# secondmind-labs/markovflow

Measured on AMD Instinct MI355X. Metric: Kalman log-lik steps/sec (BxT) at d=6, higher is better.
Workload: dtype f64; 1 GPU; KalmanFilter.log_likelihood B=1024/GPU T=10000 d=6 m=1 f64 (sum of two Matern-5/2, north-star target config); series_per_gpu=1024, state_dim=6, output_dim=1, parallelism=batch-sharded x1, one scalar RCCL all-reduce

## Files before the change

### markovflow_amd/csrc/mf_inst.hip

```cpp
#ifndef MF_D
#error "compile with -DMF_D=<state dimension>"
#endif
#include "mf_kernels.hpp"
#include "mf_kf_lds.hpp"
#include "mf_kf_x.hpp"
#include "mf_row.hpp"
#include "mf_row_par.hpp"
#include "mf_row_scan.hpp"
#include "mf_row_grad.hpp"
#include "mf_row_post.hpp"
#include "mf_row_gpr.hpp"
#include "mf_btd_par.hpp"
#include "mf_gpr_fused.hpp"
#include "mf_kl_grad.hpp"
#include "mf_post.hpp"
#include "mf_launch.hpp"

#include <cstdlib>
#include <string>
#include <type_traits>

namespace mf {
namespace {

// ... 73 lines not shown
    return v;
}

template <typename T> bool x_path() {
    static const bool on = [] { const char* e = mf_knob("MF_KF_X"); return !(e && e[0] == '0'); }();
    return on && ((sizeof(T) == 8 && D >= 7) || (sizeof(T) == 4 && D >= 9));
}
template <typename T> bool x_obs_lds(int m) {
    const int a = LdsSpike<T, D>::BYTES, b = a + LdsObs<T, D>::bytes(m);
    return (160 * 1024) / b >= 1 && ((160 * 1024) / b == (160 * 1024) / a || (160 * 1024) / b >= 4);
}
template <typename T> long x_target_lanes() {
    int w = (160 * 1024) / LdsSpike<T, D>::BYTES;
    w = w > 4 ? 4 : (w < 1 ? 1 : w);
    return 256L * 64 * w;
}

template <typename T>
int reduce_levels(RedSys<T> cur, long B, char* p, T add_const, T* out, int* info, hipStream_t st) {
    while (cur.n > red_final()) {
        const long P = cdiv(cur.n, red_chunk());
        RedSys<T> nxt = carve<T>(p, B, P);
        const long lanes = B * P;
        constexpr int x_lds = LdsSpike<T, D>::BYTES;
        if (x_path<T>())
            MF_LANE_LAUNCH((red_chunk_x_kernel<T, D>), dim3((unsigned)cdiv(lanes, 64)), dim3(64), x_lds, st, cur, nxt, B,
                               P, info);
        else
            MF_LANE_LAUNCH((red_chunk_kernel<T, D, true>), dim3((unsigned)cdiv(lanes, 64)), dim3(64), 0, st, cur, nxt,
                               B, P, info);
        cur = nxt;
    }
    MF_LANE_LAUNCH((red_final_kernel<T, D>), dim3((unsigned)cdiv(B, 64)), dim3(64), 0, st, cur, B, add_const, out,
                       info);
    return hipGetLastError() == hipSuccess ? 0 : -1000;
}

constexpr bool ROW_RED_SMALL = D >= 4 && D <= 6;
template <typename T>
int reduce_levels_row(RedSys<T> cur, long B, char* p, T add_const, T* out, int* info, hipStream_t st) {
    if constexpr ((D >= 7 || ROW_RED_SMALL) && D + 1 <= 16) {
        while (cur.n > row_red_final()) {
            const long P = cdiv(cur.n, row_red_chunk());
            RedSys<T> nxt = carve<T>(p, B, P);
            hipLaunchKernelGGL((row::red_row_kernel<T, D>), dim3((unsigned)cdiv(B * P, 4)), dim3(64), 0, st, cur, nxt, B, P, info);
            cur = nxt;
        }
        hipLaunchKernelGGL((row::red_row_final_kernel<T, D>), dim3((unsigned)cdiv(B, 4)), dim3(64), 0, st, cur, B, add_const, out,
                           info);
    }
    return hipGetLastError() == hipSuccess ? 0 : -1000;
}

template <typename T, int M, bool RSTEP> constexpr bool lds_supported() { return KfLdsCfg<T, D, M, RSTEP>::SUPPORTED; }
template <typename T> bool use_lds_kernel(long Tn, int m, int rinv_per_step) {
    static const bool force_direct = [] {
        const char* e = mf_knob("MF_KF_IMPL");
        return e && std::string(e) == "direct";
    }();
    if (force_direct || Tn < 2) return false;
    if (rinv_per_step) return m == 1 && lds_supported<T, 1, true>();
    switch (m) {
        case 1: return lds_supported<T, 1, false>();
        case 2: return lds_supported<T, 2, false>();
        case 3: return lds_supported<T, 3, false>();
        case 4: return lds_supported<T, 4, false>() && (sizeof(T) == 4 || D <= 5);
        default: return false;
    }
}
template <typename T> long lds_target_lanes(int m, int rinv_per_step) {
    auto waves = [](int lds_bytes) { const int w = (160 * 1024) / lds_bytes; return w > 4 ? 4 : (w < 1 ? 1 : w); };
    int w = 4;
    if (rinv_per_step) w = waves(KfLdsCfg<T, D, 1, true>::LDS_TOTAL);
    else if (m == 2) w = waves(KfLdsCfg<T, D, 2, false>::LDS_TOTAL);
    else if (m == 3) w = waves(KfLdsCfg<T, D, 3, false>::LDS_TOTAL);
    else if (m == 4) w = waves(KfLdsCfg<T, D, 4, false>::LDS_TOTAL);
    long lanes = 256L * 64 * w;
    const long small = sizeof(T) == 8 ? (D <= 3 ? 32768L : 65536L) : (D <= 3 ? 32768L : (D <= 5 ? 49152L : 65536L));
    return lanes < small ? lanes : small;
}

inline void lds_partition(long B, long Tn, long chunks, long& P, long& L, long target_lanes = 65536) {
    const long nt = Tn - 1;
    long want = chunks > 0 ? chunks : auto_chunks(B, nt);
    if (chunks <= 0 && target_lanes < 65536) {
        want = cdiv(target_lanes, B);
        const long maxP = nt / 4 > 0 ? nt / 4 : 1;
        if (want > maxP) want = maxP;
    }
    if (want > nt) want = nt;
    if (want < 1) want = 1;
    L = cdiv(nt, want);
    P = cdiv(nt, L);
}

enum KfPath { KF_PATH_ROW, KF_PATH_X, KF_PATH_LDS, KF_PATH_DIRECT };
template <typename T> bool row_path() {
    static const bool on = [] { const char* e = mf_knob("MF_KF_ROW"); return !(e && e[0] == '0'); }();
    return on && D + 1 <= 16 && ((sizeof(T) == 8 && D >= 7) || (sizeof(T) == 4 && D >= 9));
}
template <typename T> long row_target_rows() {
    static const long v = [] {
        const char* e = mf_knob("MF_ROW_TARGET");
        const long x = e ? std::atol(e) : 0;
        const int waves = (sizeof(T) == 4 || D <= 9) ? 3 : row::row_waves_per_simd(D);
        return x > 0 ? x : 256L * 4 * waves * 4;
    }();
    return v;
}
struct KfPlan {
    KfPath path;
    long P, L;
};
inline bool row_reduction(KfPath path) { return path == KF_PATH_ROW || (ROW_RED_SMALL && path == KF_PATH_LDS); }
template <typename T> size_t plan_ws(long B, const KfPlan& pl) {
    return row_reduction(pl.path) ? levels_ws<T>(B, pl.P, row_red_chunk(), row_red_final()) : levels_ws<T>(B, pl.P);
}
template <typename T> KfPlan kf_plan(long B, long Tn, int m, int rinv_per_step, long chunks, bool aligned16) {
    KfPlan pl{KF_PATH_DIRECT, 1, 0};
    if (row_path<T>() && Tn >= 2 && m >= 1 && m <= ROW_MAXM) {
        long P = chunks > 0 ? (chunks > Tn ? Tn : chunks) : cdiv(row_target_rows<T>(), B);
        if (chunks <= 0) {
            const long maxP = Tn / 4 > 0 ? Tn / 4 : 1;
            if (P > maxP) P = maxP;
        }
        if (row::row_offsets_fit(Tn, P, D, m, (int)sizeof(T))) {
            pl.path = KF_PATH_ROW;
            pl.P = P;
            return pl;
// ... 47 lines not shown
    const KfPlan pl = kf_plan<T>(B, Tn, m, rinv_per_step, chunks, aligned16);
    const long P = pl.P;
    if constexpr (!LANE) { if (pl.path != KF_PATH_ROW) return -100; }
    if (ws_bytes < plan_ws<T>(B, pl)) return -15;
    int dbg = 0;
#ifdef MF_EXPERIMENT
    static const int dbg_env = [] { const char* e = mf_knob("MF_KF_DEBUG"); return e ? std::atoi(e) : 0; }();
    dbg = dbg_env;
#endif
    KfArgs<T> a{B, Tn, m, mu0, cholP0, A, b, cholQ, H, y, Rinv, rinv_per_step, P, info, dbg};
    char* p = static_cast<char*>(ws);
    RedSys<T> lvl0 = carve<T>(p, B, P);
    const dim3 grid((unsigned)cdiv(B * P, 64)), block(64);
    if (ev0) (void)hipEventRecord(ev0, st);
    if (pl.path == KF_PATH_ROW) {
        if constexpr (D >= 7 && D + 1 <= 16) {
            const dim3 rgrid((unsigned)cdiv(B * P, 4));
            auto launch = [&](auto mtag) {
                constexpr int M = decltype(mtag)::value;
                if (rinv_per_step) hipLaunchKernelGGL((row::kf_row_kernel<T, D, M, true>), rgrid, block, 0, st, a, lvl0);
                else hipLaunchKernelGGL((row::kf_row_kernel<T, D, M, false>), rgrid, block, 0, st, a, lvl0);
            };
            using std::integral_constant;
            if (m == 1) launch(integral_constant<int, 1>{});
            else if (m == 2) launch(integral_constant<int, 2>{});
            else if (m == 3) launch(integral_constant<int, 3>{});
            else if (m == 4) launch(integral_constant<int, 4>{});
            else if constexpr (!LANE) {
                if (m == 5) launch(integral_constant<int, 5>{});
                else if (m == 6) launch(integral_constant<int, 6>{});
                else if (m == 7) launch(integral_constant<int, 7>{});
                else launch(integral_constant<int, 8>{});
            }
        }
    } else if (pl.path == KF_PATH_X) {
        constexpr int x_lds = LdsSpike<T, D>::BYTES;
        if (m > 1 && x_obs_lds<T>(m)) {
            const int lds = x_lds + LdsObs<T, D>::bytes(m);
            if constexpr (LANE) if (lds > 64 * 1024) {
                static const hipError_t raised = hipFuncSetAttribute(
                    reinterpret_cast<const void*>(&kf_chunk_x_kernel<T, D, true>), hipFuncAttributeMaxDynamicSharedMemorySize,
                    x_lds + LdsObs<T, D>::bytes(MF_MAXM));
                if (raised != hipSuccess) return -1000;
            }
            MF_LANE_LAUNCH((kf_chunk_x_kernel<T, D, true>), grid, block, lds, st, a, lvl0);
        } else {
            MF_LANE_LAUNCH((kf_chunk_x_kernel<T, D, false>), grid, block, x_lds, st, a, lvl0);
        }
    } else if (pl.path == KF_PATH_LDS) {
        const long L = pl.L;
        auto launch = [&](auto mtag, auto rtag) {
            constexpr int M = decltype(mtag)::value;
            constexpr bool RS = decltype(rtag)::value;
            if constexpr (KfLdsCfg<T, D, M, RS>::SUPPORTED) {
                constexpr int lds = KfLdsCfg<T, D, M, RS>::LDS_TOTAL;
                if (P > 1) MF_LANE_LAUNCH((kf_chunk_lds_kernel<T, D, M, true, RS>), grid, block, lds, st, a, L, lvl0);
                else MF_LANE_LAUNCH((kf_chunk_lds_kernel<T, D, M, false, RS>), grid, block, lds, st, a, L, lvl0);
            }
        };
        using std::integral_constant;
        if (rinv_per_step) launch(integral_constant<int, 1>{}, integral_constant<bool, true>{});
        else if (m == 1) launch(integral_constant<int, 1>{}, integral_constant<bool, false>{});
        else if (m == 2) launch(integral_constant<int, 2>{}, integral_constant<bool, false>{});
        else if (m == 3) launch(integral_constant<int, 3>{}, integral_constant<bool, false>{});
        else launch(integral_constant<int, 4>{}, integral_constant<bool, false>{});
    } else if (P > 1) {
        if (m == 1) MF_LANE_LAUNCH((kf_chunk_kernel<T, D, 1, true>), grid, block, 0, st, a, lvl0);
        else MF_LANE_LAUNCH((kf_chunk_kernel<T, D, 0, true>), grid, block, 0, st, a, lvl0);
    } else {
        if (m == 1) MF_LANE_LAUNCH((kf_chunk_kernel<T, D, 1, false>), grid, block, 0, st, a, lvl0);
        else MF_LANE_LAUNCH((kf_chunk_kernel<T, D, 0, false>), grid, block, 0, st, a, lvl0);
    }
    if (ev1) (void)hipEventRecord(ev1, st);
    if (row_reduction(pl.path)) return reduce_levels_row<T>(lvl0, B, p, add_const, out, info, st);
    return reduce_levels<T>(lvl0, B, p, add_const, out, info, st);
}

template <typename T>
int kf_loglik_plan(long B, long Tn, int m, int rinv_per_step, long chunks, int aligned16, int* path, long* P, long* L) {
    if (B < 1 || Tn < 1 || m < 1 || m > ROW_MAXM) return -1;
    const KfPlan pl = kf_plan<T>(B, Tn, m, rinv_per_step, chunks, aligned16 != 0);
    *path = (int)pl.path;
    *P = pl.P;
    *L = pl.L;
    return 0;
}

template <typename T> size_t btd_logdet_quad_ws(long B, long n, long chunks) {
    (void)chunks;
    long nn = n;
    size_t total = 256;
    while (nn > red_final()) {
        nn = cdiv(nn, red_chunk());
        total += red_bytes<T>(B, nn);
    }
    return total;
}

template <typename T>
int btd_logdet_quad(long B, long n, const T* diag, const T* sub, const T* rhs, T* out, void* ws, size_t ws_bytes,
                    int* info, long chunks, hipStream_t st) {
    if (ws_bytes < btd_logdet_quad_ws<T>(B, n, chunks) || ws == nullptr) return -9;
    RedSys<T> in;
    in.Dv = const_cast<T*>(diag);
    in.GU = nullptr;
    in.gU = nullptr;
    in.F = const_cast<T*>(sub);
    in.tv = const_cast<T*>(rhs);
// ... 1022 lines not shown
```

### markovflow_amd/csrc/mf_kf_lds.hpp

```cpp
#pragma once
#include "mf_kernels.hpp"
#ifndef MF_PUMPMASK
#define MF_PUMPMASK 63
#endif

namespace mf {

typedef int mf_v4i __attribute__((ext_vector_type(4)));

#define MF_POLICY_STR_0 ""
#define MF_POLICY_STR_1 " nt"
#define MF_POLICY_STR_2 " sc1"
#define MF_POLICY_STR_3 " sc0 sc1"
#define MF_POLICY_STR_4 " sc0"
#define MF_POLICY_CAT(n) MF_POLICY_STR_##n
#define MF_POLICY_OF(n) MF_POLICY_CAT(n)
#ifndef MF_POLW
#define MF_POLW 1
#endif
#ifndef MF_POLN
#define MF_POLN 0
#endif
#define MF_POLICY_WIDE MF_POLICY_OF(MF_POLW)
#define MF_POLICY_NARROW MF_POLICY_OF(MF_POLN)
#define MF_DMA_HEAD "s_nop 4\n\ts_mov_b32 %0, m0\n\ts_mov_b32 m0, %2\n\ts_nop 0\n\t"
#define MF_DMA_TAIL "s_mov_b32 m0, %0"
#define MF_DMA_X4(v, pol) "buffer_load_dwordx4 " v ", %1, 0 offen" pol " lds\n\t"
#define MF_DMA_X1(v, pol) "buffer_load_dword " v ", %1, 0 offen" pol " lds\n\t"
#define MF_DMA_STEP4 "s_add_u32 m0, m0, 0x400\n\ts_nop 0\n\t"
#define MF_DMA_STEP1 "s_add_u32 m0, m0, 0x100\n\ts_nop 0\n\t"
template <bool WIDE, int N> MF_DEV void dma_b128_group(mf_v4i srd, unsigned lds_addr, const unsigned* v) {
    unsigned keep;
    static_assert(N >= 1 && N <= 4, "group size");
#define MF_DMA_B128_BODY(POL)                                                                                                       \
    if constexpr (N == 1)                                                                                                           \
        asm volatile(MF_DMA_HEAD MF_DMA_X4("%3", POL) MF_DMA_TAIL : "=&s"(keep) : "s"(srd), "s"(lds_addr), "v"(v[0]) : "memory", "scc"); \
    else if constexpr (N == 2)                                                                                                      \
        asm volatile(MF_DMA_HEAD MF_DMA_X4("%3", POL) MF_DMA_STEP4 MF_DMA_X4("%4", POL) MF_DMA_TAIL                                 \
                     : "=&s"(keep) : "s"(srd), "s"(lds_addr), "v"(v[0]), "v"(v[1]) : "memory", "scc");                              \
    else if constexpr (N == 3)                                                                                                      \
        asm volatile(MF_DMA_HEAD MF_DMA_X4("%3", POL) MF_DMA_STEP4 MF_DMA_X4("%4", POL) MF_DMA_STEP4 MF_DMA_X4("%5", POL) MF_DMA_TAIL \
                     : "=&s"(keep) : "s"(srd), "s"(lds_addr), "v"(v[0]), "v"(v[1]), "v"(v[2]) : "memory", "scc");                   \
    else                                                                                                                            \
        asm volatile(MF_DMA_HEAD MF_DMA_X4("%3", POL) MF_DMA_STEP4 MF_DMA_X4("%4", POL) MF_DMA_STEP4 MF_DMA_X4("%5", POL)           \
                     MF_DMA_STEP4 MF_DMA_X4("%6", POL) MF_DMA_TAIL                                                                  \
                     : "=&s"(keep) : "s"(srd), "s"(lds_addr), "v"(v[0]), "v"(v[1]), "v"(v[2]), "v"(v[3]) : "memory", "scc");
    if (WIDE) { MF_DMA_B128_BODY(MF_POLICY_WIDE) } else { MF_DMA_B128_BODY(MF_POLICY_NARROW) }
#undef MF_DMA_B128_BODY
}
template <int N> MF_DEV void dma_b32_group(mf_v4i srd, unsigned lds_addr, const unsigned* v) {
    unsigned keep;
    static_assert(N >= 1 && N <= 4, "group size");
    if constexpr (N == 1)
        asm volatile(MF_DMA_HEAD MF_DMA_X1("%3", MF_POLICY_NARROW) MF_DMA_TAIL : "=&s"(keep) : "s"(srd), "s"(lds_addr), "v"(v[0]) : "memory", "scc");
    else if constexpr (N == 2)
        asm volatile(MF_DMA_HEAD MF_DMA_X1("%3", MF_POLICY_NARROW) MF_DMA_STEP1 MF_DMA_X1("%4", MF_POLICY_NARROW) MF_DMA_TAIL
                     : "=&s"(keep) : "s"(srd), "s"(lds_addr), "v"(v[0]), "v"(v[1]) : "memory", "scc");
    else if constexpr (N == 3)
        asm volatile(MF_DMA_HEAD MF_DMA_X1("%3", MF_POLICY_NARROW) MF_DMA_STEP1 MF_DMA_X1("%4", MF_POLICY_NARROW) MF_DMA_STEP1
                     MF_DMA_X1("%5", MF_POLICY_NARROW) MF_DMA_TAIL
                     : "=&s"(keep) : "s"(srd), "s"(lds_addr), "v"(v[0]), "v"(v[1]), "v"(v[2]) : "memory", "scc");
    else
        asm volatile(MF_DMA_HEAD MF_DMA_X1("%3", MF_POLICY_NARROW) MF_DMA_STEP1 MF_DMA_X1("%4", MF_POLICY_NARROW) MF_DMA_STEP1
                     MF_DMA_X1("%5", MF_POLICY_NARROW) MF_DMA_STEP1 MF_DMA_X1("%6", MF_POLICY_NARROW) MF_DMA_TAIL
                     : "=&s"(keep) : "s"(srd), "s"(lds_addr), "v"(v[0]), "v"(v[1]), "v"(v[2]), "v"(v[3]) : "memory", "scc");
}

template <int ROWB, typename Keep> struct Stream {
    static constexpr int UNIT = (ROWB >= 16) ? 16 : 4;
    static constexpr int UG = (ROWB + UNIT - 1) / UNIT;
    static constexpr int count_kept() { int n = 0; for (int u = 0; u < UG; ++u) n += Keep::keep(u, UNIT) ? 1 : 0; return n; }
    static constexpr int U = count_kept();
    static constexpr int NI = U;
    static constexpr int LDS_BYTES = 64 * U * UNIT;
    static constexpr bool ALL = (U == UG);
    static constexpr int global_unit(int c) {
        int n = 0;
        for (int u = 0; u < UG; ++u) if (Keep::keep(u, UNIT)) { if (n == c) return u; ++n; }
        return -1;
    }
    static constexpr int compact_unit(int gu) {
        int n = 0;
        for (int u = 0; u < gu; ++u) n += Keep::keep(u, UNIT) ? 1 : 0;
        return n;
    }
};

struct KeepAll { static constexpr bool keep(int, int) { return true; } };
template <int D, int S> struct KeepLower {
    static constexpr bool keep(int u, int unit) {
        const int lo = u * unit, hi = lo + unit;
        for (int i = 0; i < D; ++i) {
            const int a = (i * D) * S, b = (i * D + i + 1) * S;
            if (a < hi && lo < b) return true;
        }
        return false;
    }
};

constexpr unsigned MF_DMA_INVALID = 0xF0000000u;
constexpr unsigned long long MF_DMA_MAXREC = 0xE0000000ull;

template <typename St> struct DmaStream {
    unsigned vo[St::NI];
    MF_DEV void init(const char* smem, int lane, int rel_tab, int gtab) {
        const int q0 = lane / St::U, c0 = lane - q0 * St::U;
        MF_UNROLL for (int i = 0; i < St::NI; ++i) {
            const int a = (64 * i) / St::U, b = (64 * i) % St::U;
            int cu = c0 + b;
            const int carry = cu >= St::U ? 1 : 0;
            cu -= carry * St::U;
            const int row = q0 + a + carry;
            const unsigned rel = *reinterpret_cast<const unsigned*>(smem + rel_tab + row * 4);
            unsigned off;
            if (St::ALL) off = (unsigned)cu * St::UNIT;
            else off = *reinterpret_cast<const unsigned*>(smem + gtab + cu * 4);
            vo[i] = rel + off;
#ifdef MF_EXPERIMENT
            if (pack_base != 0xffffffffu && rel < MF_DMA_INVALID)
                vo[i] |= ((((pack_base + rel) >> 5) & 3u) << 29) | ((unsigned)(off / St::UNIT) << 24);
#endif
        }
    }
#ifdef MF_EXPERIMENT
    unsigned pack_base = 0xffffffffu;
    unsigned step_next = 0;
    bool skip_carried = false;
    MF_DEV unsigned exp_offset(unsigned v) const {
        if (pack_base == 0xffffffffu || v >= MF_DMA_INVALID) return v;
        const unsigned phase = ((v >> 29) + step_next) & 3u, gu = (v >> 24) & 31u, off = v & 0xffffffu;
        const bool carried = skip_carried && phase != 0u && gu < 8u - 2u * phase;
        return carried ? MF_DMA_INVALID : off;
    }
#endif
    template <int I0, int I1> MF_DEV void issue(mf_v4i srd, unsigned lds_base) const {
        constexpr int HI = I1 < St::NI ? I1 : St::NI;
        if constexpr (I0 < HI) {
            constexpr int N = (HI - I0) < 4 ? (HI - I0) : 4;
            unsigned voff[N];
            MF_UNROLL for (int k = 0; k < N; ++k) {
#ifdef MF_EXPERIMENT
                voff[k] = exp_offset(vo[I0 + k]);
#else
                voff[k] = vo[I0 + k];
#endif
            }
            if (St::UNIT == 16) dma_b128_group<(St::UG >= 8), N>(srd, lds_base + I0 * 1024, voff);
            else dma_b32_group<N>(srd, lds_base + I0 * 256, voff);
            issue<I0 + N, I1>(srd, lds_base);
        }
    }
};

MF_DEV unsigned long long uniform64(unsigned long long x) {
    const unsigned lo = (unsigned)__builtin_amdgcn_readfirstlane((int)(unsigned)x);
    const unsigned hi = (unsigned)__builtin_amdgcn_readfirstlane((int)(unsigned)(x >> 32));
    return ((unsigned long long)hi << 32) | lo;
}

MF_DEV mf_v4i make_srd(unsigned long long base, unsigned long long end, int debug = 0) {
    unsigned long long rem = end > base ? end - base : 0ull;
    if (debug & 1) rem = 0;
    if (rem > MF_DMA_MAXREC) rem = MF_DMA_MAXREC;
    mf_v4i srd;
    srd.x = __builtin_amdgcn_readfirstlane((int)(unsigned)base);
    srd.y = __builtin_amdgcn_readfirstlane((int)((unsigned)(base >> 32) & 0xffffu));
    srd.z = __builtin_amdgcn_readfirstlane((int)(unsigned)rem);
    srd.w = 0x00020000;
    return srd;
}

template <typename T, typename St> struct RowReader {
    const char* row;
    MF_DEV RowReader(const char* smem, int lds_off, int lane) : row(smem + lds_off + lane * (St::U * St::UNIT)) {}
    MF_DEV T at(int e) const {
        const int byte = e * (int)sizeof(T);
        const int gu = byte / St::UNIT;
        const int off = St::compact_unit(gu) * St::UNIT + (byte - gu * St::UNIT);
        return *reinterpret_cast<const T*>(row + off);
    }
};

template <typename T, int D, int M, bool RSTEP = false, int BG = 1> struct KfLdsCfg {
    static constexpr int S = sizeof(T);
    static constexpr int BGRP = BG;
    using StA = Stream<D * D * S, KeepAll>;
    using StC = Stream<D * D * S, KeepLower<D, S>>;
    using Stb = Stream<BG * D * S, KeepAll>;
    using StH = Stream<BG * M * D * S, KeepAll>;
    static constexpr int YG = (M == 1) ? 4 : 1;
    using Sty = Stream<YG * M * S, KeepAll>;
    using StR = Stream<M * M * S, KeepAll>;
    static constexpr bool RS = RSTEP;
    static constexpr int OFF_A = 0;
    static constexpr int OFF_C = OFF_A + StA::LDS_BYTES;
    static constexpr int OFF_b = OFF_C + StC::LDS_BYTES;
    static constexpr int OFF_H = OFF_b + Stb::LDS_BYTES;
    static constexpr int OFF_y = OFF_H + StH::LDS_BYTES;
    static constexpr int OFF_R = OFF_y + ((Sty::LDS_BYTES + 15) / 16) * 16;
    static constexpr int OFF_relA = OFF_R + (RSTEP ? ((StR::LDS_BYTES + 15) / 16) * 16 : 0);
    static constexpr int OFF_relb = OFF_relA + 256;
    static constexpr int OFF_relH = OFF_relb + 256;
    static constexpr int OFF_rely = OFF_relH + 256;
    static constexpr int OFF_relR = OFF_rely + 256;
    static constexpr int OFF_gtabC = OFF_relR + 256;
    static constexpr int LDS_TOTAL = OFF_gtabC + ((StC::U * 4 + 15) / 16) * 16;
    static constexpr bool SUPPORTED =
                                      (StA::NI + StC::NI + Stb::NI + StH::NI + Sty::NI + (RSTEP ? StR::NI : 0)) < 64 &&
                                      LDS_TOTAL <= 64 * 1024;
};

template <typename Cfg> struct KfPump {
    static constexpr int N_SMALL = Cfg::StC::NI + Cfg::Stb::NI + Cfg::StH::NI + Cfg::Sty::NI + (Cfg::RS ? Cfg::StR::NI : 0);
    static constexpr int N_BIG = Cfg::StA::NI;
    const DmaStream<typename Cfg::StA>& dA; const DmaStream<typename Cfg::StC>& dC;
    const DmaStream<typename Cfg::Stb>& db; const DmaStream<typename Cfg::StH>& dH;
    const DmaStream<typename Cfg::Sty>& dy; const DmaStream<typename Cfg::StR>& dR;
    mf_v4i sA, sC, sb, sH, sy, sR;
    unsigned lds0;
    bool more;
    bool yfetch = true;
    template <int K> MF_DEV void small() const {
        if (!((MF_PUMPMASK >> K) & 1)) return;
        small_do<K>();
    }
    template <int K> MF_DEV void small_do() const {
        if (!more) return;
        constexpr int HC = (Cfg::StC::NI + 1) / 2;
        if (K == 0) dC.template issue<0, HC>(sC, lds0 + Cfg::OFF_C);
        else {
            dC.template issue<HC, 64>(sC, lds0 + Cfg::OFF_C);
            db.template issue<0, 64>(sb, lds0 + Cfg::OFF_b);
            dH.template issue<0, 64>(sH, lds0 + Cfg::OFF_H);
            if (yfetch) dy.template issue<0, 64>(sy, lds0 + Cfg::OFF_y);
            if (Cfg::RS) dR.template issue<0, 64>(sR, lds0 + Cfg::OFF_R);
        }
    }
    template <int K> MF_DEV void all() const {
        dC.template issue<0, 64>(sC, lds0 + Cfg::OFF_C);
        db.template issue<0, 64>(sb, lds0 + Cfg::OFF_b);
        dH.template issue<0, 64>(sH, lds0 + Cfg::OFF_H);
        dy.template issue<0, 64>(sy, lds0 + Cfg::OFF_y);
        if (Cfg::RS) dR.template issue<0, 64>(sR, lds0 + Cfg::OFF_R);
        dA.template issue<0, 64>(sA, lds0 + Cfg::OFF_A);
    }
    template <int K> MF_DEV void big() const {
        if (!((MF_PUMPMASK >> (K + 2)) & 1)) return;
        big_do<K>();
    }
    MF_DEV void unpumped() const {
        if (!((MF_PUMPMASK >> 0) & 1)) small_do<0>();
        if (!((MF_PUMPMASK >> 1) & 1)) small_do<1>();
        if (!((MF_PUMPMASK >> 2) & 1)) big_do<0>();
        if (!((MF_PUMPMASK >> 3) & 1)) big_do<1>();
        if (!((MF_PUMPMASK >> 4) & 1)) big_do<2>();
        if (!((MF_PUMPMASK >> 5) & 1)) big_do<3>();
    }
    template <int K> MF_DEV void big_do() const {
        if (!more) return;
        constexpr int Q = (Cfg::StA::NI + 3) / 4;
        dA.template issue<K * Q, (K + 1) * Q>(sA, lds0 + Cfg::OFF_A);
    }
};

template <typename T, int D, int M, bool SPIKE, bool FIRST, typename Pump>
MF_DEV void kf_lds_step(Elim<T, D, SPIKE>& E, LogAcc<T>& laC, T& acc_yry, T& acc_ww, const T (&C)[D][D],
                        const T (&mvec)[D], const T (&hk)[M * D], const T (&yk)[M], const T (&Rsh)[M * M],
                        T (&Bm)[D][D], const Pump& pump, bool active, bool sep_lane) {
    const bool sep = FIRST && sep_lane, ord = active && !sep;
    T Ci[D][D], w[D], btw[D];
    if (active) {
        tri_inv_lower<T, D>(C, Ci, laC, E.bad);
        laC.renorm();
    }
    pump.template small<0>();
    if (active) {
        trimul_lower_vec<T, D>(Ci, mvec, w);
        acc_ww += dot_self<T, D>(w);
    }
    pump.template small<1>();
    pump.template big<0>();
    if (active) {
        trimul_lower_inplace<T, D, D>(Ci, Bm);
        gemv_t<T, D, D>(Bm, w, btw);
    }
    pump.template big<1>();
    if (FIRST && active && sep) {
        syrk_tn_lower<T, D, D>(Bm, E.GU, T(1));
        MF_UNROLL for (int i = 0; i < D; ++i) E.gU[i] = -btw[i];
    }
    if (ord) {
        syrk_tn_lower<T, D, D>(Bm, E.Phi, T(1));
        MF_UNROLL for (int i = 0; i < D; ++i) E.t[i] -= btw[i];
    }
    pump.template big<2>();
    if (FIRST && active && sep) {
        neg_trimulT_lower_inplace<T, D, D>(Ci, Bm);
        MF_UNROLL for (int i = 0; i < D; ++i) MF_UNROLL for (int j = 0; j < D; ++j) E.X[i][j] = Bm[i][j];
    }
    if (ord) E.eliminate_main();
    pump.template big<3>();
    if (FIRST && active && sep) {
        trimulT_self_lower<T, D>(Ci, E.Phi);
        trimulT_lower_vec<T, D>(Ci, w, E.t);
        acc_yry += Obs<T, D, M>::apply(hk, yk, Rsh, M, E.Phi, E.t);
    }
    if (ord) {
        E.eliminate_spike();
        trsm_right_lower_t<T, D, D>(E.Phi, E.Li, Bm);
        neg_trimulT_lower_inplace<T, D, D>(Ci, Bm);
        T Dn[D][D], rn[D];
        trimulT_self_lower<T, D>(Ci, Dn);
        trimulT_lower_vec<T, D>(Ci, w, rn);
        acc_yry += Obs<T, D, M>::apply(hk, yk, Rsh, M, Dn, rn);
        E.advance(Bm, Dn, rn);
    }
}

template <typename T, int D, int M, bool SPIKE, bool RSTEP = false>
__global__ void __launch_bounds__(64) kf_chunk_lds_kernel(KfArgs<T> a, long L, RedSys<T> out) {
    using Cfg = KfLdsCfg<T, D, M, RSTEP>;
    extern __shared__ __attribute__((aligned(16))) char smem[];
    const int lane = threadIdx.x;
    const long total = a.B * a.P;
    const long id_raw = (long)blockIdx.x * 64 + lane;
    const bool valid = id_raw < total;
    const long id = valid ? id_raw : total - 1;
    const long s = id / a.P, c = id % a.P;
    const long nt = a.Tn - 1;
    const long tau0 = c * L;
    long len = nt - tau0;
    if (len > L) len = L;
    if (len < 0 || !valid) len = 0;
    constexpr int S = sizeof(T);

    const unsigned long long offA = (unsigned long long)(s * nt + tau0) * (D * D * S);
    const unsigned long long offb = (unsigned long long)(s * nt + tau0) * (D * S);
    const unsigned long long offH = (unsigned long long)(s * a.Tn + tau0 + 1) * (M * D * S);
    const unsigned long long offy = (unsigned long long)(s * a.Tn + tau0 + 1) * (M * S);
    const unsigned long long offR = (unsigned long long)(s * a.Tn + tau0 + 1) * (M * M * S);
    const unsigned long long offA0 = uniform64(offA), offb0 = uniform64(offb);
    const unsigned long long offH0 = uniform64(offH), offy0 = uniform64(offy), offR0 = uniform64(offR);
    const bool rowok = valid && len > 0;
    {
        unsigned* tab = reinterpret_cast<unsigned*>(smem);
        tab[Cfg::OFF_relA / 4 + lane] = rowok ? (unsigned)(offA - offA0) : MF_DMA_INVALID;
        tab[Cfg::OFF_relb / 4 + lane] = rowok ? (unsigned)(offb - offb0) : MF_DMA_INVALID;
        tab[Cfg::OFF_relH / 4 + lane] = rowok ? (unsigned)(offH - offH0) : MF_DMA_INVALID;
        tab[Cfg::OFF_rely / 4 + lane] = rowok ? (unsigned)(offy - offy0) : MF_DMA_INVALID;
        tab[Cfg::OFF_relR / 4 + lane] = rowok ? (unsigned)(offR - offR0) : MF_DMA_INVALID;
        if (lane < Cfg::StC::U) {
            unsigned g = 0;
            MF_UNROLL for (int cc = 0; cc < Cfg::StC::U; ++cc) if (lane == cc) g = (unsigned)Cfg::StC::global_unit(cc);
            tab[Cfg::OFF_gtabC / 4 + lane] = g * Cfg::StC::UNIT;
        }
    }
    DmaStream<typename Cfg::StA> dA;
    DmaStream<typename Cfg::StC> dC;
    DmaStream<typename Cfg::Stb> db;
    DmaStream<typename Cfg::StH> dH;
    DmaStream<typename Cfg::Sty> dy;
    DmaStream<typename Cfg::StR> dR;
    unsigned long long pA = (unsigned long long)a.A + offA0, pC = (unsigned long long)a.cholQ + offA0;
    unsigned long long pb = (unsigned long long)a.b + offb0, pH = (unsigned long long)a.H + offH0;
    unsigned long long py = (unsigned long long)a.y + offy0;
    unsigned long long pR = (unsigned long long)a.Rinv + (RSTEP ? offR0 : 0ull);
    const unsigned long long eA = (unsigned long long)a.A + (unsigned long long)a.B * nt * (D * D * S);
    const unsigned long long eC = (unsigned long long)a.cholQ + (unsigned long long)a.B * nt * (D * D * S);
    const unsigned long long eb = (unsigned long long)a.b + (unsigned long long)a.B * nt * (D * S);
    const unsigned long long eH = (unsigned long long)a.H + (unsigned long long)a.B * a.Tn * (M * D * S);
    const unsigned long long ey = (unsigned long long)a.y + (unsigned long long)a.B * a.Tn * (M * S);
    const unsigned long long eR = (unsigned long long)a.Rinv + (RSTEP ? (unsigned long long)a.B * a.Tn * (M * M * S) : 0ull);
    const unsigned lds0 = (unsigned)(size_t)smem;

    Elim<T, D, SPIKE> E;
    E.init();
    LogAcc<T> laC;
    laC.init();
    T acc_yry = T(0), acc_ww = T(0);
    T Rsh[M * M];
    MF_UNROLL for (int i = 0; i < M * M; ++i) Rsh[i] = RSTEP ? (valid ? a.Rinv[(s * a.Tn) * M * M + i] : T(0)) : a.Rinv[i];
    if (valid && c == 0) {
        T C[D][D], Ci[D][D], mvec[D], w[D];
        load_lower<T, D>(a.cholP0 + s * D * D, C);
        load_vec<T, D>(a.mu0 + s * D, mvec);
        tri_inv_lower<T, D>(C, Ci, laC, E.bad);
        laC.renorm();
        trimul_lower_vec<T, D>(Ci, mvec, w);
        acc_ww += dot_self<T, D>(w);
        trimulT_self_lower<T, D>(Ci, E.Phi);
        trimulT_lower_vec<T, D>(Ci, w, E.t);
        acc_yry += Obs<T, D, M>::apply(a.H + (s * a.Tn) * M * D, a.y + (s * a.Tn) * M, Rsh, M, E.Phi, E.t);
    }

    long nsteps = len;
    MF_UNROLL for (int off = 32; off > 0; off >>= 1) {
        const long o = __shfl_xor((long long)nsteps, off);
        nsteps = o > nsteps ? o : nsteps;
    }
    nsteps = __builtin_amdgcn_readfirstlane((int)nsteps);
    asm volatile("s_waitcnt vmcnt(0) lgkmcnt(0)" ::: "memory");
#ifdef MF_EXPERIMENT
    if (a.debug & 8) {
        dA.pack_base = (unsigned)__builtin_amdgcn_readfirstlane((int)(unsigned)pA);
        dC.pack_base = (unsigned)__builtin_amdgcn_readfirstlane((int)(unsigned)pC);
    }
#endif
    dA.init(smem, lane, Cfg::OFF_relA, 0);
    dC.init(smem, lane, Cfg::OFF_relA, Cfg::OFF_gtabC);
    db.init(smem, lane, Cfg::OFF_relb, 0);
    dH.init(smem, lane, Cfg::OFF_relH, 0);
    dy.init(smem, lane, Cfg::OFF_rely, 0);
    if (RSTEP) dR.init(smem, lane, Cfg::OFF_relR, 0);

    const RowReader<T, typename Cfg::StA> rA(smem, Cfg::OFF_A, lane);
    const RowReader<T, typename Cfg::StC> rC(smem, Cfg::OFF_C, lane);
    const RowReader<T, typename Cfg::Stb> rb(smem, Cfg::OFF_b, lane);
    const RowReader<T, typename Cfg::StH> rH(smem, Cfg::OFF_H, lane);
    const RowReader<T, typename Cfg::Sty> ry(smem, Cfg::OFF_y, lane);
    const RowReader<T, typename Cfg::StR> rR(smem, Cfg::OFF_R, lane);

    using Pump = KfPump<Cfg>;

    if (nsteps > 0) {
        Pump p0{dA, dC, db, dH, dy, dR, make_srd(pA, eA, a.debug), make_srd(pC, eC, a.debug | ((a.debug >> 2) & 1)),
                make_srd(pb, eb, a.debug | ((a.debug >> 1) & 1)), make_srd(pH, eH, a.debug | ((a.debug >> 1) & 1)),
                make_srd(py, ey, a.debug | ((a.debug >> 1) & 1)), make_srd(pR, eR, a.debug | ((a.debug >> 1) & 1)), lds0, true};
        p0.template all<0>();
    }

#ifdef MF_STAMP
#define MF_STAMP_AT(var) { unsigned long long t_; asm volatile("s_memtime %0\n\ts_waitcnt lgkmcnt(0)" : "=s"(t_) :: "memory"); var = t_; }
    unsigned long long st_wait = 0, st_io = 0, st_comp = 0, ts0 = 0, ts1 = 0, ts2 = 0, ts3 = 0;
#define MF_STAMP_ACC { asm volatile("" :: "v"(E.quad), "v"(E.Phi[0][0]) : "memory"); MF_STAMP_AT(ts3) st_wait += ts1 - ts0; st_io += ts2 - ts1; st_comp += ts3 - ts2; }
#else
#define MF_STAMP_AT(var)
#define MF_STAMP_ACC
#endif
#ifdef MF_CHECKSUM
    T cs_A = 0, cs_C = 0, cs_b = 0, cs_H = 0, cs_y = 0;
#define MF_CHECKSUM_ACC if (j < len) { MF_UNROLL for (int i = 0; i < D; ++i) { cs_b += mvec[i]; MF_UNROLL for (int jj = 0; jj < D; ++jj) { cs_A += Bm[i][jj] * T(1 + i * D + jj); if (jj <= i) cs_C += C[i][jj] * T(1 + i * D + jj); } } \
        MF_UNROLL for (int i = 0; i < M * D; ++i) cs_H += hk[i] * T(1 + i); MF_UNROLL for (int i = 0; i < M; ++i) cs_y += yk[i]; }
#else
#define MF_CHECKSUM_ACC
#endif
#ifdef MF_EXPERIMENT
#define MF_EXP_STEP_NEXT { dA.step_next = dC.step_next = (unsigned)(j + 1); dA.skip_carried = dC.skip_carried = (a.debug & 8) != 0; }
#else
#define MF_EXP_STEP_NEXT
#endif
#define MF_NOPUMP_ISSUE pump.unpumped();
#define MF_KF_LDS_STEP(FIRST)                                                                                         \
    {                                                                                                                 \
        MF_STAMP_AT(ts0)                                                                                              \
        asm volatile("s_waitcnt vmcnt(0)" ::: "memory");                                                              \
        MF_STAMP_AT(ts1)                                                                                              \
        const bool more = (j + 1 < nsteps);                                                                           \
        const bool yfetch = ((j + 1) % Cfg::YG) == 0;                                                                 \
        pA += D * D * S; pC += D * D * S; pb += D * S; pH += M * D * S; if (RSTEP) pR += M * M * S;                   \
        if (yfetch) py += Cfg::YG * M * S;                                                                            \
        T C[D][D], mvec[D], hk[M * D], yk[M];                                                                         \
        MF_UNROLL for (int i = 0; i < D; ++i) MF_UNROLL for (int jj = 0; jj <= i; ++jj) C[i][jj] = rC.at(i * D + jj); \
        MF_UNROLL for (int i = 0; i < D; ++i) mvec[i] = rb.at(i);                                                     \
        MF_UNROLL for (int i = 0; i < M * D; ++i) hk[i] = rH.at(i);                                                   \
        MF_UNROLL for (int i = 0; i < M; ++i)                                                                         \
            yk[i] = *reinterpret_cast<const T*>(ry.row + ((int)(j % Cfg::YG) * M + i) * (int)sizeof(T));              \
        if (RSTEP) { MF_UNROLL for (int i = 0; i < M * M; ++i) Rsh[i] = rR.at(i); }                                    \
        T Bm[D][D];                                                                                                   \
        MF_UNROLL for (int i = 0; i < D; ++i) MF_UNROLL for (int jj = 0; jj < D; ++jj) Bm[i][jj] = rA.at(i * D + jj); \
        asm volatile("s_waitcnt lgkmcnt(0)" ::: "memory");                                                            \
        MF_CHECKSUM_ACC                                                                                               \
        MF_STAMP_AT(ts2)                                                                                              \
        const Pump pump{dA, dC, db, dH, dy, dR, make_srd(pA, eA, a.debug),                                            \
                        make_srd(pC, eC, a.debug | ((a.debug >> 2) & 1)),                                             \
                        make_srd(pb, eb, a.debug | ((a.debug >> 1) & 1)),                                             \
                        make_srd(pH, eH, a.debug | ((a.debug >> 1) & 1)),                                             \
                        make_srd(py, ey, a.debug | ((a.debug >> 1) & 1)),                                             \
                        make_srd(pR, eR, a.debug | ((a.debug >> 1) & 1)), lds0, more, yfetch};                        \
        MF_EXP_STEP_NEXT                                                                                              \
        MF_NOPUMP_ISSUE                                                                                               \
        const bool active = j < len;                                                                                  \
        kf_lds_step<T, D, M, SPIKE, FIRST>(E, laC, acc_yry, acc_ww, C, mvec, hk, yk, Rsh, Bm, pump, active, c > 0);    \
        if (E.bad && first_bad < 0) first_bad = tau0 + j;                                                             \
        MF_STAMP_ACC                                                                                                  \
    }
    long j = 0;
    long first_bad = -1;
    if (nsteps > 0) MF_KF_LDS_STEP(true)
    for (j = 1; j < nsteps; ++j) MF_KF_LDS_STEP(false)
#undef MF_KF_LDS_STEP
    asm volatile("s_waitcnt vmcnt(0)" ::: "memory");
    if (valid) {
        const T scalar = T(-0.5) * (acc_yry + acc_ww) + T(0.5) * E.quad - laC.value() - E.laL.value();
        store_chunk<T, D, SPIKE>(out, id, E, scalar);
        if (E.bad && a.info) raise_pivot(a.info, s * a.Tn + (first_bad < 0 ? tau0 : first_bad));
#ifdef MF_CHECKSUM
        out.GU[id * D * D + 0] = cs_A; out.GU[id * D * D + 1] = cs_C; out.GU[id * D * D + 2] = cs_b;
        out.gU[id * D + 0] = cs_H; out.gU[id * D + 1] = cs_y;
#endif
#ifdef MF_STAMP
        if (lane == 0) {
            out.GU[id * D * D + 0] = (T)st_wait; out.GU[id * D * D + 1] = (T)st_io; out.GU[id * D * D + 2] = (T)st_comp;
        }
#endif
    }
}

}
```

Before: 7.092 billion steps/s.

## Carry cache-line tail units of Cholesky stream across steps and overlay tables in LDS

```diff
diff --git a/markovflow_amd/csrc/mf_head_carry.hpp b/markovflow_amd/csrc/mf_head_carry.hpp
--- /dev/null
+++ b/markovflow_amd/csrc/mf_head_carry.hpp
@@ -0,0 +1,104 @@
+#pragma once
+
+namespace mf {
+
+template <int ROWB, int UNIT, typename Keep> struct HeadCarry {
+    static constexpr int LINE = 128;
+    static constexpr int MAXT = 2;
+    static constexpr int UG = (ROWB + UNIT - 1) / UNIT;
+    static constexpr int STEP = ROWB % LINE;
+    static constexpr int cand(int t) {
+        int n = 0;
+        for (int u = 0; u < UG; ++u)
+            if (Keep::keep(u, UNIT) && (u + 1) * UNIT <= LINE - 4) { if (n == t) return u; ++n; }
+        return -1;
+    }
+    static constexpr int count_cand() { int n = 0; while (n < MAXT && cand(n) >= 0) ++n; return n; }
+    static constexpr int tail_index(int u) { for (int t = 0; t < count_cand(); ++t) if (cand(t) == u) return t; return -1; }
+    static constexpr unsigned carried_units(int r) {
+        r &= LINE - 1;
+        if (r == 0) return 0u;
+        const int room = LINE - r;
+        unsigned m = 0u;
+        for (int u = 0; u < UG; ++u) {
+            if (!Keep::keep(u, UNIT) || u * UNIT >= room) continue;
+            const int t = tail_index(u);
+            if (t < 0 || (u + 1) * UNIT > room) return 0u;
+            m |= 1u << t;
+        }
+        return m;
+    }
+    static constexpr unsigned table(int t) {
+        unsigned m = 0u;
+        for (int g = 0; g < 32; ++g) if ((carried_units(4 * g) >> t) & 1u) m |= 1u << g;
+        return m;
+    }
+    static constexpr unsigned TAB0 = table(0), TAB1 = table(1);
+    static constexpr int period() { int p = 1, r = STEP; while (r % LINE) { r += STEP; ++p; } return p; }
+    static constexpr int PERIOD = (ROWB % 4 == 0) ? period() : 0;
+    static constexpr bool USABLE = ROWB % 4 == 0 && ROWB >= LINE && STEP != 0 && Keep::keep(UG - 1, UNIT) && (TAB0 | TAB1) != 0u;
+    static constexpr int NT = USABLE ? count_cand() : 0;
+    static constexpr int tail_unit(int t) { return cand(t); }
+
+    static constexpr bool carried(unsigned addr, int t) { return (((t == 0 ? TAB0 : TAB1) >> ((addr & (LINE - 1)) >> 2)) & 1u) != 0u; }
+
+    static constexpr unsigned consumer_bits(unsigned addr0) {
+        unsigned m = 0u;
+        for (int t = 0; t < NT; ++t)
+            for (int p = 0; p < PERIOD; ++p) if (carried(addr0 + (unsigned)(p * STEP), t)) m |= 1u << (t * PERIOD + p);
+        return m;
+    }
+    static constexpr unsigned producer_bits(unsigned addr0, int kind) {
+        unsigned m = 0u;
+        for (int p = 0; p < PERIOD; ++p) {
+            bool f = true;
+            if (kind >= 1 + MAXT) f = carried(addr0 + (unsigned)((p + 1) * STEP), kind - 1 - MAXT);
+            else if (kind >= 1) f = !carried(addr0 + (unsigned)(p * STEP), kind - 1);
+            if (f) m |= 1u << p;
+        }
+        return m;
+    }
+};
+
+template <int ROWB, typename Keep, bool TAIL = false> struct Stream {
+    static constexpr int UNIT = (ROWB >= 16) ? 16 : 4;
+    static constexpr int UG = (ROWB + UNIT - 1) / UNIT;
+    static constexpr int count_kept() { int n = 0; for (int u = 0; u < UG; ++u) n += Keep::keep(u, UNIT) ? 1 : 0; return n; }
+    using HC = HeadCarry<ROWB, UNIT, Keep>;
+    static constexpr int UB = count_kept();
+    static constexpr int NT = TAIL ? HC::NT : 0;
+    static constexpr int U = UB + NT;
+    static constexpr int NI = U;
+    static constexpr int LDS_BYTES = 64 * U * UNIT;
+    static constexpr bool ALL = (UB == UG) && NT == 0;
+    static constexpr int global_unit(int c) {
+        int n = 0;
+        for (int u = 0; u < UG; ++u) if (Keep::keep(u, UNIT)) { if (n == c) return u; ++n; }
+        return -1;
+    }
+    static constexpr int global_offset(int c) { return c < UB ? global_unit(c) * UNIT : ROWB + HC::tail_unit(c - UB) * UNIT; }
+    static constexpr int unit_kind(int c) {
+        if (c >= UB) return 1 + HC::MAXT + (c - UB);
+        for (int t = 0; t < NT; ++t) if (global_unit(c) == HC::tail_unit(t)) return 1 + t;
+        return 0;
+    }
+    static constexpr int compact_unit(int gu) {
+        int n = 0;
+        for (int u = 0; u < gu; ++u) n += Keep::keep(u, UNIT) ? 1 : 0;
+        return n;
+    }
+};
+
+struct KeepAll { static constexpr bool keep(int, int) { return true; } };
+template <int D, int S> struct KeepLower {
+    static constexpr bool keep(int u, int unit) {
+        const int lo = u * unit, hi = lo + unit;
+        for (int i = 0; i < D; ++i) {
+            const int a = (i * D) * S, b = (i * D + i + 1) * S;
+            if (a < hi && lo < b) return true;
+        }
+        return false;
+    }
+};
+
+}
diff --git a/markovflow_amd/csrc/mf_inst.hip b/markovflow_amd/csrc/mf_inst.hip
--- a/markovflow_amd/csrc/mf_inst.hip
+++ b/markovflow_amd/csrc/mf_inst.hip
@@ -149,7 +149,7 @@
     return hipGetLastError() == hipSuccess ? 0 : -1000;
 }
 
-template <typename T, int M, bool RSTEP> constexpr bool lds_supported() { return KfLdsCfg<T, D, M, RSTEP>::SUPPORTED; }
+template <typename T, int M, bool RSTEP> constexpr bool lds_supported() { return KfChunkCfg<T, D, M, RSTEP>::SUPPORTED; }
 template <typename T> bool use_lds_kernel(long Tn, int m, int rinv_per_step) {
     static const bool force_direct = [] {
         const char* e = mf_knob("MF_KF_IMPL");
@@ -168,10 +168,10 @@
 template <typename T> long lds_target_lanes(int m, int rinv_per_step) {
     auto waves = [](int lds_bytes) { const int w = (160 * 1024) / lds_bytes; return w > 4 ? 4 : (w < 1 ? 1 : w); };
     int w = 4;
-    if (rinv_per_step) w = waves(KfLdsCfg<T, D, 1, true>::LDS_TOTAL);
-    else if (m == 2) w = waves(KfLdsCfg<T, D, 2, false>::LDS_TOTAL);
-    else if (m == 3) w = waves(KfLdsCfg<T, D, 3, false>::LDS_TOTAL);
-    else if (m == 4) w = waves(KfLdsCfg<T, D, 4, false>::LDS_TOTAL);
+    if (rinv_per_step) w = waves(KfChunkCfg<T, D, 1, true>::LDS_TOTAL);
+    else if (m == 2) w = waves(KfChunkCfg<T, D, 2, false>::LDS_TOTAL);
+    else if (m == 3) w = waves(KfChunkCfg<T, D, 3, false>::LDS_TOTAL);
+    else if (m == 4) w = waves(KfChunkCfg<T, D, 4, false>::LDS_TOTAL);
     long lanes = 256L * 64 * w;
     const long small = sizeof(T) == 8 ? (D <= 3 ? 32768L : 65536L) : (D <= 3 ? 32768L : (D <= 5 ? 49152L : 65536L));
     return lanes < small ? lanes : small;
@@ -325,8 +325,8 @@
         auto launch = [&](auto mtag, auto rtag) {
             constexpr int M = decltype(mtag)::value;
             constexpr bool RS = decltype(rtag)::value;
-            if constexpr (KfLdsCfg<T, D, M, RS>::SUPPORTED) {
-                constexpr int lds = KfLdsCfg<T, D, M, RS>::LDS_TOTAL;
+            if constexpr (KfChunkCfg<T, D, M, RS>::SUPPORTED) {
+                constexpr int lds = KfChunkCfg<T, D, M, RS>::LDS_TOTAL;
                 if (P > 1) MF_LANE_LAUNCH((kf_chunk_lds_kernel<T, D, M, true, RS>), grid, block, lds, st, a, L, lvl0);
                 else MF_LANE_LAUNCH((kf_chunk_lds_kernel<T, D, M, false, RS>), grid, block, lds, st, a, L, lvl0);
             }
diff --git a/markovflow_amd/csrc/mf_kf_lds.hpp b/markovflow_amd/csrc/mf_kf_lds.hpp
--- a/markovflow_amd/csrc/mf_kf_lds.hpp
+++ b/markovflow_amd/csrc/mf_kf_lds.hpp
@@ -1,5 +1,7 @@
 #pragma once
 #include "mf_kernels.hpp"
+#include "mf_head_carry.hpp"
+#include <type_traits>
 #ifndef MF_PUMPMASK
 #define MF_PUMPMASK 63
 #endif
@@ -66,45 +68,22 @@
                      : "=&s"(keep) : "s"(srd), "s"(lds_addr), "v"(v[0]), "v"(v[1]), "v"(v[2]), "v"(v[3]) : "memory", "scc");
 }
 
-template <int ROWB, typename Keep> struct Stream {
-    static constexpr int UNIT = (ROWB >= 16) ? 16 : 4;
-    static constexpr int UG = (ROWB + UNIT - 1) / UNIT;
-    static constexpr int count_kept() { int n = 0; for (int u = 0; u < UG; ++u) n += Keep::keep(u, UNIT) ? 1 : 0; return n; }
-    static constexpr int U = count_kept();
-    static constexpr int NI = U;
-    static constexpr int LDS_BYTES = 64 * U * UNIT;
-    static constexpr bool ALL = (U == UG);
-    static constexpr int global_unit(int c) {
-        int n = 0;
-        for (int u = 0; u < UG; ++u) if (Keep::keep(u, UNIT)) { if (n == c) return u; ++n; }
-        return -1;
-    }
-    static constexpr int compact_unit(int gu) {
-        int n = 0;
-        for (int u = 0; u < gu; ++u) n += Keep::keep(u, UNIT) ? 1 : 0;
-        return n;
-    }
-};
-
-struct KeepAll { static constexpr bool keep(int, int) { return true; } };
-template <int D, int S> struct KeepLower {
-    static constexpr bool keep(int u, int unit) {
-        const int lo = u * unit, hi = lo + unit;
-        for (int i = 0; i < D; ++i) {
-            const int a = (i * D) * S, b = (i * D + i + 1) * S;
-            if (a < hi && lo < b) return true;
-        }
-        return false;
-    }
-};
 
 constexpr unsigned MF_DMA_INVALID = 0xF0000000u;
 constexpr unsigned long long MF_DMA_MAXREC = 0xE0000000ull;
 
+template <typename St, typename = void> struct StreamTail { static constexpr int NT = 0, PERIOD = 1; };
+template <typename St> struct StreamTail<St, std::enable_if_t<(St::NT > 0)>> { static constexpr int NT = St::NT, PERIOD = St::HC::PERIOD; };
+
 template <typename St> struct DmaStream {
+    using TL = StreamTail<St>;
     unsigned vo[St::NI];
-    MF_DEV void init(const char* smem, int lane, int rel_tab, int gtab) {
+    static constexpr int PB = TL::PERIOD;
+    static constexpr int FW = TL::NT > 0 ? (St::NI * PB + 31) / 32 : 1;
+    unsigned fm[FW];
+    MF_DEV void init(const char* smem, int lane, int rel_tab, int gtab, unsigned base_lo = 0u) {
         const int q0 = lane / St::U, c0 = lane - q0 * St::U;
+        if constexpr (TL::NT > 0) { MF_UNROLL for (int w = 0; w < FW; ++w) fm[w] = 0u; }
         MF_UNROLL for (int i = 0; i < St::NI; ++i) {
             const int a = (64 * i) / St::U, b = (64 * i) % St::U;
             int cu = c0 + b;
@@ -116,6 +95,15 @@
             if (St::ALL) off = (unsigned)cu * St::UNIT;
             else off = *reinterpret_cast<const unsigned*>(smem + gtab + cu * 4);
             vo[i] = rel + off;
+            if constexpr (TL::NT > 0) {
+                static_assert(PB < 32 && 32 % PB == 0, "an instruction's schedule bits do not straddle two words");
+                int kind = 0;
+                MF_UNROLL for (int cc = 0; cc < St::U; ++cc) if (St::unit_kind(cc) != 0 && cu == cc) kind = St::unit_kind(cc);
+                unsigned bits = (1u << PB) - 1u;
+                MF_UNROLL for (int kk = 1; kk <= 2 * St::HC::MAXT; ++kk)
+                    if (kind == kk) bits = St::HC::producer_bits(base_lo + rel, kk);
+                fm[(i * PB) / 32] |= bits << ((i * PB) % 32);
+            }
 #ifdef MF_EXPERIMENT
             if (pack_base != 0xffffffffu && rel < MF_DMA_INVALID)
                 vo[i] |= ((((pack_base + rel) >> 5) & 3u) << 29) | ((unsigned)(off / St::UNIT) << 24);
@@ -133,7 +121,7 @@
         return carried ? MF_DMA_INVALID : off;
     }
 #endif
-    template <int I0, int I1> MF_DEV void issue(mf_v4i srd, unsigned lds_base) const {
+    template <int I0, int I1, bool SCHED = false> MF_DEV void issue(mf_v4i srd, unsigned lds_base, unsigned phase = 0u) const {
         constexpr int HI = I1 < St::NI ? I1 : St::NI;
         if constexpr (I0 < HI) {
             constexpr int N = (HI - I0) < 4 ? (HI - I0) : 4;
@@ -144,10 +132,12 @@
 #else
                 voff[k] = vo[I0 + k];
 #endif
+                if constexpr (SCHED && TL::NT > 0)
+                    voff[k] = ((fm[((I0 + k) * PB) / 32] >> (((I0 + k) * PB) % 32 + phase)) & 1u) ? voff[k] : MF_DMA_INVALID;
             }
             if (St::UNIT == 16) dma_b128_group<(St::UG >= 8), N>(srd, lds_base + I0 * 1024, voff);
             else dma_b32_group<N>(srd, lds_base + I0 * 256, voff);
-            issue<I0 + N, I1>(srd, lds_base);
+            issue<I0 + N, I1, SCHED>(srd, lds_base, phase);
         }
     }
 };
@@ -179,36 +169,50 @@
         const int off = St::compact_unit(gu) * St::UNIT + (byte - gu * St::UNIT);
         return *reinterpret_cast<const T*>(row + off);
     }
+    MF_DEV T tail_at(int t, int k) const { return *reinterpret_cast<const T*>(row + (St::UB + t) * St::UNIT + k * (int)sizeof(T)); }
 };
 
-template <typename T, int D, int M, bool RSTEP = false, int BG = 1> struct KfLdsCfg {
+template <typename T, int D, int M, bool RSTEP = false, int BG = 1, bool CARRY = false> struct KfLdsCfg {
     static constexpr int S = sizeof(T);
     static constexpr int BGRP = BG;
     using StA = Stream<D * D * S, KeepAll>;
-    using StC = Stream<D * D * S, KeepLower<D, S>>;
+    using StC0 = Stream<D * D * S, KeepLower<D, S>>;
+    using StCT = Stream<D * D * S, KeepLower<D, S>, true>;
     using Stb = Stream<BG * D * S, KeepAll>;
     using StH = Stream<BG * M * D * S, KeepAll>;
     static constexpr int YG = (M == 1) ? 4 : 1;
     using Sty = Stream<YG * M * S, KeepAll>;
     using StR = Stream<M * M * S, KeepAll>;
     static constexpr bool RS = RSTEP;
+    static constexpr int QUARTER_CU = (160 * 1024) / 4;
+    static constexpr int TABLE_BYTES = 5 * 256 + ((StCT::U * 4 + 15) / 16) * 16;
+    static constexpr int IMAGE_T = StA::LDS_BYTES + StCT::LDS_BYTES + Stb::LDS_BYTES + StH::LDS_BYTES + ((Sty::LDS_BYTES + 15) / 16) * 16 +
+                                   (RSTEP ? ((StR::LDS_BYTES + 15) / 16) * 16 : 0);
+    static constexpr bool TAIL = CARRY && StCT::NT > 0 && !StC0::ALL && StCT::NI * StCT::HC::PERIOD <= 64 &&
+                                 StCT::NT * StCT::HC::PERIOD <= 32 && IMAGE_T <= QUARTER_CU && TABLE_BYTES <= IMAGE_T &&
+                                 (StA::NI + StCT::NI + Stb::NI + StH::NI + Sty::NI + (RSTEP ? StR::NI : 0)) < 64;
+    using StC = Stream<D * D * S, KeepLower<D, S>, TAIL>;
     static constexpr int OFF_A = 0;
     static constexpr int OFF_C = OFF_A + StA::LDS_BYTES;
     static constexpr int OFF_b = OFF_C + StC::LDS_BYTES;
     static constexpr int OFF_H = OFF_b + Stb::LDS_BYTES;
     static constexpr int OFF_y = OFF_H + StH::LDS_BYTES;
     static constexpr int OFF_R = OFF_y + ((Sty::LDS_BYTES + 15) / 16) * 16;
-    static constexpr int OFF_relA = OFF_R + (RSTEP ? ((StR::LDS_BYTES + 15) / 16) * 16 : 0);
+    static constexpr int IMAGE_END = OFF_R + (RSTEP ? ((StR::LDS_BYTES + 15) / 16) * 16 : 0);
+    static constexpr int OFF_relA = TAIL ? 0 : IMAGE_END;
     static constexpr int OFF_relb = OFF_relA + 256;
     static constexpr int OFF_relH = OFF_relb + 256;
     static constexpr int OFF_rely = OFF_relH + 256;
     static constexpr int OFF_relR = OFF_rely + 256;
     static constexpr int OFF_gtabC = OFF_relR + 256;
-    static constexpr int LDS_TOTAL = OFF_gtabC + ((StC::U * 4 + 15) / 16) * 16;
+    static constexpr int LDS_TOTAL = TAIL ? IMAGE_END : OFF_gtabC + ((StC::U * 4 + 15) / 16) * 16;
     static constexpr bool SUPPORTED =
                                       (StA::NI + StC::NI + Stb::NI + StH::NI + Sty::NI + (RSTEP ? StR::NI : 0)) < 64 &&
                                       LDS_TOTAL <= 64 * 1024;
 };
+
+template <typename T, int D, int M, bool RSTEP = false> using KfChunkCfg = KfLdsCfg<T, D, M, RSTEP, 1, true>;
+static_assert(KfChunkCfg<double, 6, 1>::TAIL && KfChunkCfg<double, 6, 1>::LDS_TOTAL <= 40960, "fp64 d = 6: four wavefronts per CU");
 
 template <typename Cfg> struct KfPump {
     static constexpr int N_SMALL = Cfg::StC::NI + Cfg::Stb::NI + Cfg::StH::NI + Cfg::Sty::NI + (Cfg::RS ? Cfg::StR::NI : 0);
@@ -220,6 +224,7 @@
     unsigned lds0;
     bool more;
     bool yfetch = true;
+    unsigned cphase = 0;
     template <int K> MF_DEV void small() const {
         if (!((MF_PUMPMASK >> K) & 1)) return;
         small_do<K>();
@@ -227,9 +232,9 @@
     template <int K> MF_DEV void small_do() const {
         if (!more) return;
         constexpr int HC = (Cfg::StC::NI + 1) / 2;
-        if (K == 0) dC.template issue<0, HC>(sC, lds0 + Cfg::OFF_C);
+        if (K == 0) dC.template issue<0, HC, true>(sC, lds0 + Cfg::OFF_C, cphase);
         else {
-            dC.template issue<HC, 64>(sC, lds0 + Cfg::OFF_C);
+            dC.template issue<HC, 64, true>(sC, lds0 + Cfg::OFF_C, cphase);
             db.template issue<0, 64>(sb, lds0 + Cfg::OFF_b);
             dH.template issue<0, 64>(sH, lds0 + Cfg::OFF_H);
             if (yfetch) dy.template issue<0, 64>(sy, lds0 + Cfg::OFF_y);
@@ -319,7 +324,7 @@
 
 template <typename T, int D, int M, bool SPIKE, bool RSTEP = false>
 __global__ void __launch_bounds__(64) kf_chunk_lds_kernel(KfArgs<T> a, long L, RedSys<T> out) {
-    using Cfg = KfLdsCfg<T, D, M, RSTEP>;
+    using Cfg = KfChunkCfg<T, D, M, RSTEP>;
     extern __shared__ __attribute__((aligned(16))) char smem[];
     const int lane = threadIdx.x;
     const long total = a.B * a.P;
@@ -351,8 +356,8 @@
         tab[Cfg::OFF_relR / 4 + lane] = rowok ? (unsigned)(offR - offR0) : MF_DMA_INVALID;
         if (lane < Cfg::StC::U) {
             unsigned g = 0;
-            MF_UNROLL for (int cc = 0; cc < Cfg::StC::U; ++cc) if (lane == cc) g = (unsigned)Cfg::StC::global_unit(cc);
-            tab[Cfg::OFF_gtabC / 4 + lane] = g * Cfg::StC::UNIT;
+            MF_UNROLL for (int cc = 0; cc < Cfg::StC::U; ++cc) if (lane == cc) g = (unsigned)Cfg::StC::global_offset(cc);
+            tab[Cfg::OFF_gtabC / 4 + lane] = g;
         }
     }
     DmaStream<typename Cfg::StA> dA;
@@ -407,11 +412,17 @@
     }
 #endif
     dA.init(smem, lane, Cfg::OFF_relA, 0);
-    dC.init(smem, lane, Cfg::OFF_relA, Cfg::OFF_gtabC);
+    dC.init(smem, lane, Cfg::OFF_relA, Cfg::OFF_gtabC, (unsigned)pC);
     db.init(smem, lane, Cfg::OFF_relb, 0);
     dH.init(smem, lane, Cfg::OFF_relH, 0);
     dy.init(smem, lane, Cfg::OFF_rely, 0);
     if (RSTEP) dR.init(smem, lane, Cfg::OFF_relR, 0);
+    asm volatile("s_waitcnt lgkmcnt(0)" ::: "memory");
+    using HC = typename Cfg::StC::HC;
+    constexpr int NTAIL = Cfg::StC::NT, CPER = NTAIL > 0 ? HC::PERIOD : 1, UEL = Cfg::StC::UNIT / S;
+    const unsigned cbits = NTAIL > 0 ? HC::consumer_bits((unsigned)((unsigned long long)a.cholQ + offA)) : 0u;
+    T cv[NTAIL > 0 ? NTAIL : 1][UEL];
+    MF_UNROLL for (int t = 0; t < (NTAIL > 0 ? NTAIL : 1); ++t) MF_UNROLL for (int k = 0; k < UEL; ++k) cv[t][k] = T(0);
 
     const RowReader<T, typename Cfg::StA> rA(smem, Cfg::OFF_A, lane);
     const RowReader<T, typename Cfg::StC> rC(smem, Cfg::OFF_C, lane);
@@ -461,6 +472,17 @@
         if (yfetch) py += Cfg::YG * M * S;                                                                            \
         T C[D][D], mvec[D], hk[M * D], yk[M];                                                                         \
         MF_UNROLL for (int i = 0; i < D; ++i) MF_UNROLL for (int jj = 0; jj <= i; ++jj) C[i][jj] = rC.at(i * D + jj); \
+        if constexpr (NTAIL > 0) {                                                                                    \
+               \
+               \
+            MF_UNROLL for (int t = 0; t < NTAIL; ++t) {                                                               \
+                const bool got = !(FIRST) && ((cbits >> (t * CPER + (int)(j & (CPER - 1)))) & 1u) != 0u;              \
+                MF_UNROLL for (int i = 0; i < D; ++i) MF_UNROLL for (int jj = 0; jj <= i; ++jj)                       \
+                    if (((i * D + jj) * S) / Cfg::StC::UNIT == HC::tail_unit(t))                                      \
+                        C[i][jj] = got ? cv[t][(i * D + jj) - HC::tail_unit(t) * UEL] : C[i][jj];                     \
+                MF_UNROLL for (int k = 0; k < UEL; ++k) cv[t][k] = rC.tail_at(t, k);                                  \
+            }                                                                                                         \
+        }                                                                                                             \
         MF_UNROLL for (int i = 0; i < D; ++i) mvec[i] = rb.at(i);                                                     \
         MF_UNROLL for (int i = 0; i < M * D; ++i) hk[i] = rH.at(i);                                                   \
         MF_UNROLL for (int i = 0; i < M; ++i)                                                                         \
@@ -476,7 +498,8 @@
                         make_srd(pb, eb, a.debug | ((a.debug >> 1) & 1)),                                             \
                         make_srd(pH, eH, a.debug | ((a.debug >> 1) & 1)),                                             \
                         make_srd(py, ey, a.debug | ((a.debug >> 1) & 1)),                                             \
-                        make_srd(pR, eR, a.debug | ((a.debug >> 1) & 1)), lds0, more, yfetch};                        \
+                        make_srd(pR, eR, a.debug | ((a.debug >> 1) & 1)), lds0, more, yfetch,                         \
+                        (unsigned)((j + 1) & (CPER - 1))};                                                            \
         MF_EXP_STEP_NEXT                                                                                              \
         MF_NOPUMP_ISSUE                                                                                               \
         const bool active = j < len;                                                                                  \
```

Result: faster. 7.805 billion steps/s, median of 6 (+10.1%).
